# 0Setsuna0/SoftbodyUnity

Measured on AMD Instinct MI355X. Metric: particle-substeps/sec, higher is better.
Workload: dtype f32

## Files before the change

include/softbody_debug.h:

```cpp
#ifndef SOFTBODY_MI355X_DEBUG_H
#define SOFTBODY_MI355X_DEBUG_H

#include "softbody.h"

#ifdef __cplusplus
extern "C" {
#endif

#define SB_DEBUG_NO_COMM  1u
#define SB_DEBUG_LOOPBACK 2u

#define SB_TUNE_NO_MASS_PALETTE   (1u << 0)
#define SB_TUNE_NO_UNIFORM_MASS   (1u << 1)
#define SB_TUNE_NO_PALETTE        (1u << 2)
#define SB_TUNE_NO_WAVE_ITEMS     (1u << 3)
#define SB_TUNE_NO_LANE_PACK      (1u << 4)
#define SB_TUNE_NO_COST_ORDER     (1u << 5)
#define SB_TUNE_NO_FUSED_UNPACK   (1u << 6)
#define SB_TUNE_PEER_COARSE       (1u << 7)
#define SB_TUNE_NO_LAZY_TICK      (1u << 8)
#define SB_TUNE_NO_PACK           (1u << 9)
#define SB_TUNE_NO_PEEK           (1u << 10)
#define SB_TUNE_NO_KIN_FUSE       (1u << 11)
#define SB_TUNE_NO_WIDE_SLOTS     (1u << 12)
#define SB_TUNE_AUTO_PREFER_OVERLAP (1u << 13)
#define SB_TUNE_NO_AUTO_CALIBRATION (1u << 14)
typedef struct {
    uint32_t flags;
    int32_t tile_lanes;
    int32_t quad_lanes;
    int32_t narrow_min_tiles;
    int32_t store_through_max_tiles;
    int32_t store_through_large;
    int32_t peek_min_tiles;
    int32_t lds_pad_bytes;
    int32_t win_dwords;
    int32_t prev_offset_bytes;
    int32_t reserved[6];
} sb_tuning;
void sb_tuning_default(sb_tuning *t);
int sb_set_tuning(sb_solver *s, const sb_tuning *t);

int sb_profile_begin(sb_solver *s);
int sb_profile_end(sb_solver *s, float *elapsed_ms_out);
int sb_step_profiled(sb_solver *s, float dt, int32_t substeps, float *slot_ms_out, int32_t *slot_launches_out,
                     int32_t n_slots);
typedef struct {
    int64_t exchanges;
    double pack_ms, transport_ms, total_ms;
    double exposed_wait_ms;
} sb_exchange_timing;
int sb_debug_exchange_timing(sb_solver *s, int32_t enabled);
int sb_debug_exchange_timing_read(sb_solver *s, sb_exchange_timing *out);

int sb_debug_launch(sb_solver *s, float dt, int32_t substeps, int32_t it, int32_t gcolour);
int sb_debug_halo_pack(sb_solver *s, int32_t slot, float *host_out, int64_t capacity_floats, int64_t *count_floats_out);
int sb_debug_halo_unpack(sb_solver *s, int32_t slot, const float *host_in, int64_t count_floats);

typedef struct {
    int64_t tiles_checked, groups_checked, constraints_checked;
    int64_t errors[6];
    int32_t first_stage;
    int32_t first_tile, first_group, first_kind;
} sb_validate_report;
int sb_debug_validate(sb_solver *s, int32_t inject_fault, sb_validate_report *out);

int sb_debug_last_words(int32_t fd, const char *text, int64_t len, int32_t exit_code);

#ifdef __cplusplus
}
#endif
#endif
```

softbodyunity_amd/csrc/abi.hip:

```cpp
#include "solver_internal.hpp"

using namespace sbi;

extern "C" {

void sb_desc_default(sb_desc *d) {
    if (!d) return;
    std::memset(d, 0, sizeof(*d));
    d->world = 1;
    d->gravity[1] = -9.81f;
    d->tile_particles = 0;
    d->use_graph = 1;
}

int sb_create(const sb_desc *desc, sb_solver **out) {
    if (!desc || !out) return fail(SB_ERR_INVALID_ARG, "sb_create: null argument");
    *out = nullptr;
    return guarded([&]() -> int {
        sb_desc d = *desc;
        if (d.world <= 0) d.world = 1;
        if (d.rank < 0 || d.rank >= d.world) return fail(SB_ERR_INVALID_ARG, "sb_create: rank out of range");
        if (!(d.damping >= 0.0f)) return fail(SB_ERR_INVALID_ARG, "sb_create: damping must be >= 0");
        if (d.tile_particles > sbp::kMaxTileLocal) return fail(SB_ERR_INVALID_ARG, "sb_create: tile_particles too large");
        if (d.partition < SB_PARTITION_AUTO || d.partition > SB_PARTITION_RCB) return fail(SB_ERR_INVALID_ARG, "sb_create: partition must be SB_PARTITION_AUTO, _BLOCKS or _RCB");
        if (d.plan_flags & ~kPlanFlagsAll) return fail(SB_ERR_INVALID_ARG, "sb_create: unknown bit in plan_flags");
        if (d.halo_transport != SB_TRANSPORT_RCCL && d.halo_transport != SB_TRANSPORT_PEER) return fail(SB_ERR_INVALID_ARG, "sb_create: halo_transport must be SB_TRANSPORT_RCCL or _PEER");
        if (d.halo_schedule < SB_SCHEDULE_AUTO || d.halo_schedule > SB_SCHEDULE_OVERLAP_GRAPH) return fail(SB_ERR_INVALID_ARG, "sb_create: halo_schedule must be one of SB_SCHEDULE_*");
        if (d.debug_flags & ~(SB_DEBUG_NO_COMM | SB_DEBUG_LOOPBACK)) return fail(SB_ERR_INVALID_ARG, "sb_create: unknown bit in debug_flags");
        if (d.reserved[0] || d.reserved[1] || d.reserved[2]) return fail(SB_ERR_INVALID_ARG, "sb_create: reserved fields must be 0 (zero-initialise sb_desc or call sb_desc_default)");
        int ndev = 0;
        hipError_t e = hipGetDeviceCount(&ndev);
        if (e != hipSuccess || ndev <= 0)
            return fail(SB_ERR_NO_DEVICE, "sb_create: no HIP device (this plugin has no CPU path)");
        if (d.device < 0 || d.device >= ndev) return fail(SB_ERR_NO_DEVICE, "sb_create: device ordinal out of range");
        hipDeviceProp_t prop;
        HIP_CHECK(hipGetDeviceProperties(&prop, d.device));
        if (std::strncmp(prop.gcnArchName, "gfx950", 6) != 0)
            return fail(SB_ERR_NO_DEVICE, std::string("sb_create: device is ") + prop.gcnArchName + ", kernels are built for gfx950 only");
        HIP_CHECK(hipSetDevice(d.device));
        auto s = std::make_unique<sb_solver>();
        s->desc = d;
        s->peer.enabled = d.world > 1 && d.halo_transport == SB_TRANSPORT_PEER;
        s->loopback = d.world > 1 && (d.debug_flags & SB_DEBUG_LOOPBACK) != 0;
        HIP_CHECK(hipStreamCreateWithFlags(&s->stream, hipStreamNonBlocking));
        HIP_CHECK(hipEventCreate(&s->ev0));
        HIP_CHECK(hipEventCreate(&s->ev1));
        *out = s.release();
        return SB_OK;
    });
}

void sb_tuning_default(sb_tuning *t) {
    if (!t) return;
    std::memset(t, 0, sizeof(*t));
    t->store_through_max_tiles = -1;
    t->peek_min_tiles = -1;
}

int sb_set_tuning(sb_solver *s, const sb_tuning *t) {
    if (!s || !t) return fail(SB_ERR_INVALID_ARG, "sb_set_tuning: null argument");
    if (s->finalized) return fail(SB_ERR_STATE, "sb_set_tuning after sb_finalize");
    constexpr uint32_t kAll = (SB_TUNE_NO_AUTO_CALIBRATION << 1) - 1u;
    if (t->flags & ~kAll) return fail(SB_ERR_INVALID_ARG, "sb_set_tuning: unknown bit in flags");
    for (int32_t r : t->reserved) if (r) return fail(SB_ERR_INVALID_ARG, "sb_set_tuning: reserved fields must be 0 (sb_tuning_default)");
    if (t->tile_lanes != 0 && t->tile_lanes != 128 && t->tile_lanes != 256 && t->tile_lanes != 512) return fail(SB_ERR_INVALID_ARG, "sb_set_tuning: tile_lanes must be 0, 128, 256 or 512");
    if (t->quad_lanes != 0 && t->quad_lanes != 256 && t->quad_lanes != 512) return fail(SB_ERR_INVALID_ARG, "sb_set_tuning: quad_lanes must be 0, 256 or 512");
    if (t->prev_offset_bytes < 0 || (t->prev_offset_bytes & 15)) return fail(SB_ERR_INVALID_ARG, "sb_set_tuning: prev_offset_bytes must be a non-negative multiple of 16");
    if (t->narrow_min_tiles < 0 || t->store_through_max_tiles < -1 || t->peek_min_tiles < -1 || t->lds_pad_bytes < 0 || t->win_dwords < 0 || (t->store_through_large & ~3))
        return fail(SB_ERR_INVALID_ARG, "sb_set_tuning: value out of range");
    s->tune_flags = t->flags;
    s->lazy_tick = !(t->flags & SB_TUNE_NO_LAZY_TICK);
    s->pack_tiles = !(t->flags & SB_TUNE_NO_PACK);
    s->peek_enabled = !(t->flags & SB_TUNE_NO_PEEK);
    s->kin_fuse = !(t->flags & SB_TUNE_NO_KIN_FUSE);
    s->tile_lanes = t->tile_lanes;
    s->quad_lanes = t->quad_lanes ? t->quad_lanes : 512;
    if (t->narrow_min_tiles > 0) s->narrow_min_tiles = t->narrow_min_tiles;
    if (t->store_through_max_tiles >= 0) s->store_through_max_tiles = t->store_through_max_tiles;
    s->store_through_large = t->store_through_large;
    if (t->peek_min_tiles >= 0) s->peek_min_tiles = t->peek_min_tiles;
    s->lds_pad = (size_t)t->lds_pad_bytes;
    s->win_dwords_cap = t->win_dwords;
    s->prev_offset_bytes = t->prev_offset_bytes;
    return SB_OK;
}

int sb_destroy(sb_solver *s) {
    if (!s) return fail(SB_ERR_INVALID_ARG, "sb_destroy: null handle");
    (void)hipSetDevice(s->desc.device);
    delete s;
    return SB_OK;
}

int sb_set_particles(sb_solver *s, const float *pos, const float *vel, const float *inv_mass, int32_t n) {
    if (!s || !pos || !inv_mass || n <= 0) return fail(SB_ERR_INVALID_ARG, "sb_set_particles: bad argument");
    if (s->finalized) return fail(SB_ERR_STATE, "sb_set_particles after sb_finalize");
    return guarded([&]() -> int {
        for (int32_t p = 0; p < n; ++p) if (!(inv_mass[p] >= 0.0f)) return fail(SB_ERR_INVALID_ARG, "sb_set_particles: inverse mass must be >= 0");
        s->n = n;
        s->pos.assign(pos, pos + 3 * (size_t)n);
        if (vel) s->vel.assign(vel, vel + 3 * (size_t)n); else s->vel.assign(3 * (size_t)n, 0.0f);
        s->invm.assign(inv_mass, inv_mass + n);
        return SB_OK;
    });
}

int sb_set_rest_positions(sb_solver *s, const float *rest, int32_t n) {
    if (!s || !rest) return fail(SB_ERR_INVALID_ARG, "sb_set_rest_positions: bad argument");
    if (s->finalized) return fail(SB_ERR_STATE, "sb_set_rest_positions after sb_finalize");
    if (n != s->n) return fail(SB_ERR_INVALID_ARG, "sb_set_rest_positions: n differs from sb_set_particles");
    return guarded([&]() -> int { s->rest.assign(rest, rest + 3 * (size_t)n); return SB_OK; });
}

static int set_cons(sb_solver *s, const char *who, const int32_t *idx, const float *rest, int32_t m, float compliance,
                    int type, int nv, int nrest) {
// ... 274 lines not shown
    return SB_OK;
}

int finalize_agree(sb_solver *s, int local_rc) {
    const int W = s->desc.world;
    const size_t rec = (size_t)W + 2;
    const std::string my_error = local_rc ? std::string(last_error_text()) : std::string();
    std::vector<uint64_t> mine = agreement_record(s, local_rc != SB_OK);
    std::vector<uint64_t> all((size_t)W * rec);
    const int rc = guarded([&]() -> int {
        int r0 = set_device(s); if (r0) return r0;
        DevBuf<uint64_t> d_all; int64_t acct = 0;
        d_all.alloc((size_t)W * rec, acct);
        HIP_CHECK(hipMemcpy(d_all.p + (size_t)s->desc.rank * rec, mine.data(), rec * sizeof(uint64_t), hipMemcpyHostToDevice));
        NCCL_CHECK(rccl().AllGather(d_all.p + (size_t)s->desc.rank * rec, d_all.p, rec * sizeof(uint64_t), ncclUint8, s->comm, s->stream));
        HIP_CHECK(hipStreamSynchronize(s->stream));
        HIP_CHECK(hipMemcpy(all.data(), d_all.p, all.size() * sizeof(uint64_t), hipMemcpyDeviceToHost));
        return SB_OK;
    });
    if (local_rc) return fail(local_rc, my_error);
    if (rc) return rc;
    return check_agreement(all, W, s->desc.rank);
}

int finalize_link(sb_solver *s) {
    return guarded([&]() -> int {
        int rc = set_device(s); if (rc) return rc;
        if (s->peer.enabled && s->desc.world > 1) {
            if (s->loopback) {
                peer_link(s);
            } else if (s->comm) {
                const int W = s->desc.world;
                hipIpcMemHandle_t mine;
                HIP_CHECK(hipIpcGetMemHandle(&mine, s->peer.mailbox));
                DevBuf<uint8_t> d_all; int64_t acct = 0;
                d_all.alloc((size_t)W * sizeof(mine), acct);
                HIP_CHECK(hipMemcpy(d_all.p + (size_t)s->desc.rank * sizeof(mine), &mine, sizeof(mine), hipMemcpyHostToDevice));
                NCCL_CHECK(rccl().AllGather(d_all.p + (size_t)s->desc.rank * sizeof(mine), d_all.p, sizeof(mine), ncclUint8, s->comm, s->stream));
                HIP_CHECK(hipStreamSynchronize(s->stream));
                std::vector<hipIpcMemHandle_t> all((size_t)W);
                HIP_CHECK(hipMemcpy(all.data(), d_all.p, (size_t)W * sizeof(mine), hipMemcpyDeviceToHost));
                for (int r = 0; r < W; ++r) {
                    if (r == s->desc.rank) continue;
                    bool needed = false;
                    for (const auto &H : s->halos) for (int pr : H->peers) needed |= pr == r;
                    if (!needed) continue;
                    void *p = nullptr;
                    HIP_CHECK(hipIpcOpenMemHandle(&p, all[(size_t)r], hipIpcMemLazyEnablePeerAccess));
                    s->peer.remote[(size_t)r] = (uint32_t *)p; s->peer.opened[(size_t)r] = 1;
                }
                peer_link(s);
            }
        }
        if (std::getenv("SB_PRINT_ALLOC"))
            std::fprintf(stderr, "[alloc] pos3 %p prev %p vel %p wf %p w8 %p T0.stream %p T1.stream %p T0.tiles %p T1.tiles %p\n", (void *)s->d_pos3.p, (void *)s->d_prev.p,
                         (void *)s->d_vel.p, (void *)s->d_wf.p, (void *)s->d_w8.p, (void *)s->tiling[0].stream.p, (void *)s->tiling[1].stream.p,
                         (void *)s->tiling[0].tiles.p, (void *)s->tiling[1].tiles.p);
        HIP_CHECK(hipDeviceSynchronize());
        std::vector<float>().swap(s->pos); std::vector<float>().swap(s->vel); std::vector<float>().swap(s->rest);
        std::vector<int32_t>().swap(s->dist_ij); std::vector<int32_t>().swap(s->vol_ijkl); std::vector<int32_t>().swap(s->bend_ijkl);
        std::vector<float>().swap(s->dist_rest); std::vector<float>().swap(s->vol_rest); std::vector<float>().swap(s->bend_rest);
        s->finalized = true;
        return SB_OK;
    });
}

}

extern "C" {

int sb_finalize(sb_solver *s) {
    if (!s) return fail(SB_ERR_INVALID_ARG, "sb_finalize: null handle");
    if (s->finalized) return fail(SB_ERR_STATE, "sb_finalize called twice");
    if (s->n <= 0) return fail(SB_ERR_STATE, "sb_finalize before sb_set_particles");
    const bool no_comm = (s->desc.debug_flags & SB_DEBUG_NO_COMM) != 0;
    if (s->desc.world > 1 && !s->comm && !s->peer.enabled && !no_comm)
        return fail(SB_ERR_STATE, "sb_finalize: world > 1 needs sb_comm_init first (or halo_transport = SB_TRANSPORT_PEER with sb_peer_connect)");
    int rc = guarded([&]() -> int { return finalize_local(s); });
    if (s->desc.world > 1 && s->comm && !s->loopback) rc = finalize_agree(s, rc);
    if (rc) return rc;
    return finalize_link(s);
}

int sb_synchronize(sb_solver *s) {
    if (!s) return fail(SB_ERR_INVALID_ARG, "sb_synchronize: null handle");
    return guarded([&]() -> int {
        int rc = set_device(s); if (rc) return rc;
        flush_deferred(s);
        HIP_CHECK(hipStreamSynchronize(s->stream));
        check_peer_error(s);
        return SB_OK;
    });
}

int sb_get_owner(sb_solver *s, int32_t *owner, int32_t n) {
    if (!s || !owner) return fail(SB_ERR_INVALID_ARG, "sb_get_owner: null argument");
    if (!s->finalized) return fail(SB_ERR_STATE, "sb_get_owner before sb_finalize");
    if (n != s->n) return fail(SB_ERR_INVALID_ARG, "sb_get_owner: n mismatch");
    std::memcpy(owner, s->plan->plan.owner_of_old.data(), (size_t)n * sizeof(int32_t));
    return SB_OK;
}

int sb_profile_begin(sb_solver *s) {
    if (!s) return fail(SB_ERR_INVALID_ARG, "sb_profile_begin: null handle");
    return guarded([&]() -> int {
        int rc = set_device(s); if (rc) return rc;
        HIP_CHECK(hipEventRecord(s->ev0, s->stream));
        return SB_OK;
    });
}
// ... 78 lines not shown
```

softbodyunity_amd/csrc/solver_internal.hpp:

```cpp
#pragma once
#include <hip/hip_runtime.h>
#include <rccl/rccl.h>
#include <dlfcn.h>

#include <algorithm>
#include <array>
#include <atomic>
#include <chrono>
#include <climits>
#include <cmath>
#include <cstdio>
#include <cstdlib>
#include <cstring>
#include <limits>
#include <map>
#include <memory>
#include <mutex>
#include <type_traits>
#include <stdexcept>
#include <string>
#include <utility>
#include <vector>

#include "../../include/softbody.h"
// ... 32 lines not shown
    decltype(&ncclGroupEnd) GroupEnd = nullptr;
    decltype(&ncclSend) Send = nullptr;
    decltype(&ncclRecv) Recv = nullptr;
    decltype(&ncclAllGather) AllGather = nullptr;
    bool ok() const { return handle != nullptr; }
};
RcclApi &rccl(bool required = true);
#define NCCL_CHECK(expr)                                                                                  \
    do {                                                                                                  \
        ncclResult_t r_ = (expr);                                                                         \
        if (r_ != ncclSuccess)                                                                            \
            throw HipError(SB_ERR_RCCL, std::string(#expr) + ": " + rccl().GetErrorString(r_));          \
    } while (0)

int hip_runtime_version();
bool capture_overlap_ok();

template <class T>
struct DevBuf {
    T *p = nullptr;
    T *base = nullptr;
    size_t count = 0;
    DevBuf() = default;
    DevBuf(const DevBuf &) = delete;
    DevBuf &operator=(const DevBuf &) = delete;
    DevBuf(DevBuf &&o) noexcept : p(o.p), base(o.base), count(o.count) { o.p = o.base = nullptr; o.count = 0; }
    DevBuf &operator=(DevBuf &&o) noexcept { if (this != &o) { free(); p = o.p; base = o.base; count = o.count; o.p = o.base = nullptr; o.count = 0; } return *this; }
    void alloc(size_t n, int64_t &acct, size_t lead_elems = 0) {
        free();
        count = n;
        if (n) { HIP_CHECK(hipMalloc((void **)&base, (n + lead_elems) * sizeof(T))); p = base + lead_elems; acct += (int64_t)((n + lead_elems) * sizeof(T)); }
    }
    void upload(const std::vector<T> &h, int64_t &acct) {
        alloc(h.size(), acct);
        if (!h.empty()) HIP_CHECK(hipMemcpy(p, h.data(), h.size() * sizeof(T), hipMemcpyHostToDevice));
    }
    void free() { if (base) { (void)hipFree(base); } base = nullptr; p = nullptr; count = 0; }
    ~DevBuf() { free(); }
};

struct DevHalo {
    std::vector<int> peers;
    std::vector<int32_t> send_off, recv_off;
    DevBuf<int32_t> send_idx, recv_idx;
    bool active() const { return !peers.empty(); }
};

struct DevTiling {
    int32_t n_tiles = 0;
    size_t lds_bytes = 0;
    int64_t n_slots = 0;
    int64_t staged_particles = 0;
    int64_t stream_bytes = 0;
    int32_t max_local = 0, win_dwords = 4, pal_dwords = 0, rounds_dwords = 0;
    int32_t n_boundary = 0;
    bool has_quads = false;
    int32_t item_waves = 0;
    int32_t packed_lanes = 0;
    int64_t n_packed_tiles = 0;
    DevBuf<sbk::TileDesc> tiles;
    DevBuf<int2> runs_overflow;
    DevBuf<uint32_t> stream;
    DevBuf<int32_t> gather;
};

struct DevGColour {
    int type = 0;
    int32_t count = 0;
    DevBuf<int2> ij;
    DevBuf<int4> quad;
    DevBuf<float> rest;
    DevBuf<float2> rest2;
};

}

namespace sbi {

enum class StepKind : uint8_t { Tile, T2Layer, GColour, Exchange, ForkExchange, JoinExchange };
enum class TileRange : uint8_t { All, T0Boundary, T0Interior, T1Interior, T1Boundary };
struct TickStep {
    StepKind kind;
    TileRange range;
    bool kin;
    int it, substeps;
    int index;
};
struct TickShape { int substeps; bool fuse, defer_last, kin; };

struct ExchangeTimer {
    bool enabled = false;
    std::vector<hipEvent_t> pending, join_pending, free_list;
    void mark(hipStream_t st, bool join = false);
    ~ExchangeTimer();
};

}

using sbi::DevBuf; using sbi::DevGColour; using sbi::DevHalo; using sbi::DevTiling;

struct sb_plan {
    sbp::Plan plan;
    sbp::LocalPlan local;
    bool owns_local = true;
};

// ... 230 lines not shown
```

softbodyunity_amd/csrc/tables.hip:

```cpp
#include "solver_internal.hpp"

namespace sbi {

sbp::Input make_input(const float *rest, int32_t n, const int32_t *d, int64_t md, const int32_t *v, int64_t mv,
                      const int32_t *b, int64_t mb) {
    sbp::Input in;
    in.rest = rest; in.n = n; in.dist_ij = d; in.m_d = md; in.vol = v; in.m_v = mv; in.bend = b; in.m_b = mb;
    return in;
}

sbp::Domain to_domain(const sb_domain &d) {
    sbp::Domain D;
    D.set = true; D.n_global = d.n_global; D.ell = d.spacing; D.fill = d.fill > 0 && d.fill <= 1 ? d.fill : 1.0;
    for (int a = 0; a < 3; ++a) { D.lo[a] = d.lo[a]; D.hi[a] = d.hi[a]; }
    return D;
}
sbp::Opts plan_opts(int rank, int world, const int32_t dims[3], int32_t tile_particles, int32_t partition, uint32_t plan_flags,
                    int64_t m_v, int64_t m_b, const sb_domain *domain) {
    sbp::Opts o;
    if (domain) {
        o.domain = to_domain(*domain);
        if (domain->four_vertex_constraints) m_v += 1;
    }
    o.rank = rank; o.world = world <= 0 ? 1 : world;
// ... 410 lines not shown
                        } else {
                            stream.push_back(idx);
                            stream.push_back(rb);
                        }
                    }
                }
                while ((stream.size() - s0) & 3) stream.push_back(0);
                for (int t = 1; t < 3; ++t)
                    for (const Part &pt : R.parts) {
                        const uint32_t b = (uint32_t)base[pt.member], b2 = b | (b << 16);
                        const int64_t kb = pt.first_q + (t == 2 ? pt.cnt[1] : 0);
                        for (int64_t k = kb; k < kb + pt.cnt[t]; ++k) {
                            if (G.t_quad_type[k] != t) throw std::runtime_error("internal: group layout");
                            Q.has_quads = true;
                            stream.push_back(G.t_quad[2 * k] + b2); stream.push_back(G.t_quad[2 * k + 1] + b2);
                            const int32_t id = G.t_quad_id[k];
                            if (t == 1) { volatile float r6 = 6.0f * s->vol_rest[id]; stream.push_back(fbits(r6)); stream.push_back(0); }
                            else { stream.push_back(fbits(s->bend_rest[2 * (size_t)id])); stream.push_back(fbits(s->bend_rest[2 * (size_t)id + 1])); }
                        }
                    }
            }
            td.s_len = (uint32_t)(stream.size() - s0);
            if (!td.packed_lanes) max_data = std::max(max_data, td.s_len - td.s_hdr);
            tiles.push_back(td);
        }
        });
        std::vector<sbk::TileDesc> tiles;
        std::vector<int2> overflow;
        std::vector<uint32_t> stream;
        std::vector<int32_t> dev_gather;
        int32_t max_local = 0, max_pal = 0, max_rounds = 0;
        uint32_t max_data = 4;
        {
            size_t nt = 0, no = 0, ns = 0, ng = 0;
            for (const Piece &Q : pieces) { nt += Q.tiles.size(); no += Q.overflow.size(); ns += Q.stream.size(); ng += Q.dev_gather.size(); }
            if (ns > 0xfffffff0ull) throw std::runtime_error("tile constraint stream exceeds 2^32 dwords");
            tiles.reserve(nt); overflow.reserve(no); stream.reserve(ns); dev_gather.reserve(ng);
            for (Piece &Q : pieces) {
                for (sbk::TileDesc td : Q.tiles) {
                    td.s_begin += (uint32_t)stream.size();
                    td.run_overflow += (int32_t)overflow.size();
                    td.gather_begin += (int32_t)dev_gather.size();
                    tiles.push_back(td);
                }
                overflow.insert(overflow.end(), Q.overflow.begin(), Q.overflow.end());
                stream.insert(stream.end(), Q.stream.begin(), Q.stream.end());
                dev_gather.insert(dev_gather.end(), Q.dev_gather.begin(), Q.dev_gather.end());
                max_local = std::max(max_local, Q.max_local); max_pal = std::max(max_pal, Q.max_pal);
                max_rounds = std::max(max_rounds, Q.max_rounds); max_data = std::max(max_data, Q.max_data);
                D.has_quads |= Q.has_quads;
                Piece().tiles.swap(Q.tiles); std::vector<uint32_t>().swap(Q.stream);
            }
        }
        if (!(s->tune_flags & SB_TUNE_NO_COST_ORDER)) {
            constexpr int32_t kCostOrderMaxTiles = 2048;
            const int32_t n = (int32_t)tiles.size();
            std::vector<std::pair<int32_t, int32_t>> ranges;
            if (tl == 2) ranges = s->t2_layer_range;
            else if ((s->overlap_halo || s->calib.state == 1) && D.n_boundary > 0 && D.n_boundary < n) {
                const int32_t cut = tl == 0 ? D.n_boundary : n - D.n_boundary;
                ranges = {{0, cut}, {cut, n}};
            } else ranges = {{0, n}};
            for (const auto &rg : ranges) {
                const int32_t nr = rg.second - rg.first;
                if (nr < 2 || nr > kCostOrderMaxTiles) continue;
                std::vector<int32_t> cost((size_t)nr), idx((size_t)nr);
                for (int32_t k = 0; k < nr; ++k) {
                    const sbk::TileDesc &td = tiles[(size_t)(rg.first + k)];
                    int32_t c = 0;
                    for (int32_t r = 0; r < td.n_rounds; ++r) {
                        const uint32_t w = stream[(size_t)td.s_begin + (size_t)r];
                        const int32_t nd = (int32_t)(w & 1023u), nv = (int32_t)((w >> 10) & 1023u), nb = (int32_t)((w >> 20) & 1023u);
                        if (D.has_quads) {
                            const int nw = std::max(1, (int)D.item_waves ? (int)D.item_waves : 4);
                            c += std::max(1, (((nd + 63) >> 6) + ((nv + 15) >> 4) + ((nb + 3) >> 2) + nw - 1) / nw) + (nb > 0 ? 1 : 0);
                        }
                        else c += std::max(1, (nd + sbk::kRoundSlots - 1) / sbk::kRoundSlots);
                    }
                    cost[(size_t)k] = c; idx[(size_t)k] = k;
                }
                const auto mm = std::minmax_element(cost.begin(), cost.end());
                if ((int64_t)*mm.second * 4 <= (int64_t)*mm.first * 5) continue;
                std::stable_sort(idx.begin(), idx.end(), [&](int32_t a, int32_t b2) { return cost[(size_t)a] > cost[(size_t)b2]; });
                std::vector<sbk::TileDesc> placed((size_t)nr);
                const int32_t xq = nr >> 3, xr = nr & 7;
                for (int32_t w = 0; w < nr; ++w) {
                    const int32_t xcd = w & 7;
                    const int32_t pos = (xcd < xr ? xcd * (xq + 1) : xr * (xq + 1) + (xcd - xr) * xq) + (w >> 3);
                    placed[(size_t)pos] = tiles[(size_t)(rg.first + idx[(size_t)w])];
                }
                std::copy(placed.begin(), placed.end(), tiles.begin() + rg.first);
            }
        }
        D.n_tiles = (int32_t)tiles.size();
        D.n_packed_tiles = n_packed_tiles.load();
        D.max_local = std::max(max_local, 1);
        D.win_dwords = (int32_t)std::min<uint32_t>(max_data, 8192u);
        if (s->win_dwords_cap > 0) D.win_dwords = std::max(1024, std::min(D.win_dwords, s->win_dwords_cap) & ~3);
        D.pal_dwords = (max_pal + 3) & ~3;
        D.rounds_dwords = std::min(sbk::kMaxRoundsLds, (max_rounds + 3) & ~3);
        D.lds_bytes = (size_t)D.max_local * sizeof(float4) + (size_t)D.rounds_dwords * 4 + (size_t)D.pal_dwords * 4 + (size_t)D.win_dwords * 4 + 16;
        D.n_slots = 0;
        for (size_t ci = 0; ci < LT.tile_ids.size(); ++ci) {
            const sbp::Tile &T = G.tiles[LT.tile_ids[ci]];
            D.n_slots += (T.d_end - T.d_begin) + (T.q_end - T.q_begin);
        }
        D.staged_particles = 0;
        for (const sbk::TileDesc &td : tiles) D.staged_particles += td.n_local;
        D.stream_bytes = (int64_t)stream.size() * 4;
        D.tiles.upload(tiles, s->dev_bytes); D.runs_overflow.upload(overflow, s->dev_bytes);
        D.stream.upload(stream, s->dev_bytes);
        D.gather.upload(dev_gather, s->dev_bytes);
    }
    for (const sbp::LocalGColour &LG : L.gcolours) {
        auto D = std::make_unique<DevGColour>();
        D->type = LG.type; D->count = (int32_t)LG.id.size();
        if (LG.type == 0) {
            std::vector<int2> ij(LG.id.size()); std::vector<float> rest(LG.id.size());
            for (size_t k = 0; k < LG.id.size(); ++k) { ij[k] = make_int2(LG.idx[2 * k], LG.idx[2 * k + 1]); rest[k] = s->dist_rest[LG.id[k]]; }
            D->ij.upload(ij, s->dev_bytes); D->rest.upload(rest, s->dev_bytes);
        } else {
            std::vector<int4> q(LG.id.size()); std::vector<float2> rest(LG.id.size());
            for (size_t k = 0; k < LG.id.size(); ++k) {
                q[k] = make_int4(LG.idx[4 * k], LG.idx[4 * k + 1], LG.idx[4 * k + 2], LG.idx[4 * k + 3]);
                const int32_t id = LG.id[k];
                if (LG.type == 1) { volatile float r6 = 6.0f * s->vol_rest[id]; rest[k] = make_float2(r6, 0.0f); }
                else rest[k] = make_float2(s->bend_rest[2 * (size_t)id], s->bend_rest[2 * (size_t)id + 1]);
            }
            D->quad.upload(q, s->dev_bytes); D->rest2.upload(rest, s->dev_bytes);
        }
        s->gcolours.push_back(std::move(D));
    }
    size_t max_send = 0, max_recv = 0;
    for (size_t slot = 0; slot < L.halo.size(); ++slot) {
        const sbp::HaloSlot &H = L.halo[slot];
        auto D = std::make_unique<DevHalo>();
        std::vector<int32_t> sidx, ridx;
        D->send_off.push_back(0); D->recv_off.push_back(0);
        for (int peer = 0; peer < L.world; ++peer) {
            if (H.send_idx[peer].empty() && H.recv_idx[peer].empty()) continue;
            D->peers.push_back(peer);
            sidx.insert(sidx.end(), H.send_idx[peer].begin(), H.send_idx[peer].end());
            ridx.insert(ridx.end(), H.recv_idx[peer].begin(), H.recv_idx[peer].end());
            D->send_off.push_back((int32_t)sidx.size()); D->recv_off.push_back((int32_t)ridx.size());
        }
        D->send_idx.upload(sidx, s->dev_bytes); D->recv_idx.upload(ridx, s->dev_bytes);
        const size_t fl = slot == 1 ? 6 : 3;
        max_send = std::max(max_send, sidx.size() * fl); max_recv = std::max(max_recv, ridx.size() * fl);
        s->halos.push_back(std::move(D));
    }
    s->d_sendbuf.alloc(max_send, s->dev_bytes);
    s->d_recvbuf.alloc(max_recv, s->dev_bytes);
    if (max_recv) HIP_CHECK(hipMemset(s->d_recvbuf.p, 0, max_recv * sizeof(float)));
    s->fused_unpack = false;
    if (L.world > 1 && !s->peer.enabled && P.tiling && P.gcolours.empty() && P.t2_layers.empty() && !s->tiling[1].has_quads &&
        s->halos.size() > 1 && !(s->tune_flags & SB_TUNE_NO_FUSED_UNPACK)) {
        std::vector<int32_t> ridx;
        for (int peer = 0; peer < L.world; ++peer) ridx.insert(ridx.end(), L.halo[1].recv_idx[(size_t)peer].begin(), L.halo[1].recv_idx[(size_t)peer].end());
        bool identity = (int64_t)ridx.size() == s->n_local - s->n_owned && !ridx.empty();
        for (size_t k = 0; identity && k < ridx.size(); ++k) identity = ridx[k] == (int32_t)(s->n_owned + (int64_t)k);
        s->fused_unpack = identity;
    }
// ... 45 lines not shown
```

softbodyunity_amd/native.py:

```python
import ctypes as C
import os

import numpy as np

_HERE = os.path.dirname(os.path.abspath(__file__))
_VARIANT = os.environ.get("SB_LIB_VARIANT", "")
LIB_PATH = os.path.join(_HERE, f"libsoftbody_mi355x{'_' + _VARIANT if _VARIANT else ''}.so")

SB_UNIQUE_ID_BYTES = 128
SB_IPC_HANDLE_BYTES = 64
SB_OK = 0
SB_PARTITION_AUTO, SB_PARTITION_BLOCKS, SB_PARTITION_RCB = 0, 1, 2
SB_PLAN_NO_T2, SB_PLAN_NO_THIRD_LIST, SB_PLAN_NO_CLUSTER_LAYERS, SB_PLAN_NO_MIXED_GROUPS, SB_PLAN_NO_BANK_ORDER, SB_PLAN_NO_TILE_MERGE = 1, 2, 4, 8, 16, 32
SB_TRANSPORT_RCCL, SB_TRANSPORT_PEER = 0, 1
SB_SCHEDULE_AUTO, SB_SCHEDULE_SERIAL_EAGER, SB_SCHEDULE_SERIAL_GRAPH, SB_SCHEDULE_OVERLAP_EAGER, SB_SCHEDULE_OVERLAP_GRAPH = 0, 1, 2, 3, 4
SB_DEBUG_NO_COMM, SB_DEBUG_LOOPBACK = 1, 2
SB_GROUP_WALK = 1
SB_GROUP_WHOLE_MESH = 2
(SB_TUNE_NO_MASS_PALETTE, SB_TUNE_NO_UNIFORM_MASS, SB_TUNE_NO_PALETTE, SB_TUNE_NO_WAVE_ITEMS, SB_TUNE_NO_LANE_PACK, SB_TUNE_NO_COST_ORDER,
 SB_TUNE_NO_FUSED_UNPACK, SB_TUNE_PEER_COARSE, SB_TUNE_NO_LAZY_TICK, SB_TUNE_NO_PACK, SB_TUNE_NO_PEEK, SB_TUNE_NO_KIN_FUSE,
 SB_TUNE_NO_WIDE_SLOTS, SB_TUNE_AUTO_PREFER_OVERLAP, SB_TUNE_NO_AUTO_CALIBRATION) = (1 << k for k in range(15))
SB_ERR_INVALID_ARG, SB_ERR_STATE, SB_ERR_NO_DEVICE, SB_ERR_HIP, SB_ERR_RCCL, SB_ERR_NOMEM, SB_ERR_UNSUPPORTED = \
    -1, -2, -3, -4, -5, -6, -7


class SbDesc(C.Structure):
    _fields_ = [("device", C.c_int32), ("rank", C.c_int32), ("world", C.c_int32), ("part_dims", C.c_int32 * 3),
                ("gravity", C.c_float * 3), ("damping", C.c_float), ("tile_particles", C.c_int32),
                ("use_graph", C.c_int32), ("partition", C.c_int32), ("plan_flags", C.c_uint32),
                ("halo_transport", C.c_int32), ("halo_schedule", C.c_int32), ("debug_flags", C.c_uint32),
                ("reserved", C.c_int32 * 3)]


class SbTuning(C.Structure):
    _fields_ = [("flags", C.c_uint32), ("tile_lanes", C.c_int32), ("quad_lanes", C.c_int32), ("narrow_min_tiles", C.c_int32),
                ("store_through_max_tiles", C.c_int32), ("store_through_large", C.c_int32), ("peek_min_tiles", C.c_int32),
                ("lds_pad_bytes", C.c_int32), ("win_dwords", C.c_int32), ("prev_offset_bytes", C.c_int32), ("reserved", C.c_int32 * 6)]


class SbExchangeTiming(C.Structure):
    _fields_ = [("exchanges", C.c_int64), ("pack_ms", C.c_double), ("transport_ms", C.c_double), ("total_ms", C.c_double), ("exposed_wait_ms", C.c_double)]


class SbStats(C.Structure):
    _fields_ = [("n_particles_owned", C.c_int64), ("n_particles_local", C.c_int64),
                ("n_constraints_local", C.c_int64 * 3), ("n_tilings", C.c_int32), ("n_global_colours", C.c_int32),
                ("n_tiles", C.c_int64 * 2), ("tile_constraints", C.c_int64 * 2), ("constraints_in_tiles", C.c_int64),
                ("constraints_in_global", C.c_int64), ("halo_particles_t1", C.c_int64),
                ("halo_particles_global", C.c_int64), ("device_bytes", C.c_int64),
                ("n_t2_layers", C.c_int64), ("n_t2_tiles", C.c_int64), ("t2_constraints", C.c_int64),
                ("launch_bytes", C.c_int64 * 5), ("partition", C.c_int32), ("halo_peers", C.c_int32),
                ("partition_cost", C.c_int64), ("partition_cost_max", C.c_int64), ("partition_cost_total", C.c_int64),
                ("halo_particles_recv", C.c_int64), ("plan_hash", C.c_uint64), ("halo_schedule", C.c_int32),
                ("halo_unpack_fused", C.c_int32), ("readback_peeks", C.c_int64), ("readback_peek_tiles", C.c_int64), ("ticks_fused", C.c_int64), ("ticks_fused_kinematic", C.c_int64), ("lane_packed_tiles", C.c_int64 * 2),
                ("halo_auto_state", C.c_int32), ("halo_auto_ticks", C.c_int32), ("halo_auto_ms", C.c_double * 2)]

    def as_dict(self):
        out = {}
        for name, _ in self._fields_:
            v = getattr(self, name)
            out[name] = list(v) if hasattr(v, "__len__") else v
        return out


class SbValidateReport(C.Structure):
    _fields_ = [("tiles_checked", C.c_int64), ("groups_checked", C.c_int64), ("constraints_checked", C.c_int64), ("errors", C.c_int64 * 6),
                ("first_stage", C.c_int32), ("first_tile", C.c_int32), ("first_group", C.c_int32), ("first_kind", C.c_int32)]


class SbDomain(C.Structure):
    _fields_ = [("n_global", C.c_int64), ("lo", C.c_double * 3), ("hi", C.c_double * 3), ("spacing", C.c_double), ("fill", C.c_double),
                ("four_vertex_constraints", C.c_int32), ("reserved", C.c_int32)]


# ... 131 lines not shown
        _lib = L
    return _lib


def check(rc):
    if rc != SB_OK:
        raise SoftbodyError(rc, lib().sb_last_error().decode("utf-8", "replace"))


def ptr(a):
    return None if a is None else a.ctypes.data_as(C.c_void_p)


def f32(a, shape=None):
    a = np.ascontiguousarray(a, dtype=np.float32)
    return a if shape is None else a.reshape(shape)


def i32(a, shape=None):
    a = np.ascontiguousarray(a, dtype=np.int32)
    return a if shape is None else a.reshape(shape)


_PLAN_FLAG_ENV = (("SB_NO_T2", SB_PLAN_NO_T2), ("SB_NO_THIRD_LIST", SB_PLAN_NO_THIRD_LIST),
                  ("SB_NO_CLUSTER_LAYERS", SB_PLAN_NO_CLUSTER_LAYERS), ("SB_NO_MIXED_GROUPS", SB_PLAN_NO_MIXED_GROUPS),
                  ("SB_NO_BANK_ORDER", SB_PLAN_NO_BANK_ORDER), ("SB_NO_TILE_MERGE", SB_PLAN_NO_TILE_MERGE))


def plan_flags_from_env():
    lists = int(os.environ.get("SB_BALANCED_LISTS", "0") or 0) & 3
    return sum(bit for name, bit in _PLAN_FLAG_ENV if os.environ.get(name)) | (lists << 8)


def halo_transport_from_env():
    return SB_TRANSPORT_PEER if os.environ.get("SB_HALO_TRANSPORT") == "peer" else SB_TRANSPORT_RCCL


def halo_schedule_from_env():
    overlap, graph = bool(os.environ.get("SB_HALO_OVERLAP")), bool(os.environ.get("SB_GRAPH_RCCL"))
    if not overlap and not graph:
        return SB_SCHEDULE_AUTO
    return (SB_SCHEDULE_OVERLAP_GRAPH if graph else SB_SCHEDULE_OVERLAP_EAGER) if overlap else SB_SCHEDULE_SERIAL_GRAPH


def debug_flags_from_env():
    return (SB_DEBUG_NO_COMM if os.environ.get("SB_TEST_NO_COMM") else 0) | (SB_DEBUG_LOOPBACK if os.environ.get("SB_TEST_LOOPBACK") else 0)


_TUNE_FLAG_ENV = (("SB_NO_MASS_PALETTE", SB_TUNE_NO_MASS_PALETTE), ("SB_NO_UNIFORM_MASS", SB_TUNE_NO_UNIFORM_MASS), ("SB_NO_PALETTE", SB_TUNE_NO_PALETTE),
                  ("SB_NO_WAVE_ITEMS", SB_TUNE_NO_WAVE_ITEMS), ("SB_NO_LANE_PACK", SB_TUNE_NO_LANE_PACK), ("SB_NO_COST_ORDER", SB_TUNE_NO_COST_ORDER),
                  ("SB_NO_FUSED_UNPACK", SB_TUNE_NO_FUSED_UNPACK), ("SB_PEER_COARSE", SB_TUNE_PEER_COARSE), ("SB_NO_LAZY_TICK", SB_TUNE_NO_LAZY_TICK),
                  ("SB_NO_PACK", SB_TUNE_NO_PACK), ("SB_NO_PEEK", SB_TUNE_NO_PEEK), ("SB_NO_KIN_FUSE", SB_TUNE_NO_KIN_FUSE),
                  ("SB_NO_WIDE_SLOTS", SB_TUNE_NO_WIDE_SLOTS), ("SB_AUTO_PREFER_OVERLAP", SB_TUNE_AUTO_PREFER_OVERLAP),
                  ("SB_NO_AUTO_CALIBRATION", SB_TUNE_NO_AUTO_CALIBRATION))
_TUNE_INT_ENV = (("SB_TILE_LANES", "tile_lanes"), ("SB_QUAD_LANES", "quad_lanes"), ("SB_NARROW_MIN_TILES", "narrow_min_tiles"),
                 ("SB_STORE_THROUGH_MAX_TILES", "store_through_max_tiles"), ("SB_STORE_THROUGH_LARGE", "store_through_large"),
                 ("SB_PEEK_MIN_TILES", "peek_min_tiles"), ("SB_LDS_PAD", "lds_pad_bytes"), ("SB_WIN_DWORDS", "win_dwords"),
                 ("SB_PREV_OFFSET", "prev_offset_bytes"))


def tuning_from_env():
    t = SbTuning()
    lib().sb_tuning_default(C.byref(t))
    any_set = False
    for name, bit in _TUNE_FLAG_ENV:
        if os.environ.get(name):
            t.flags |= bit; any_set = True
    for name, field in _TUNE_INT_ENV:
        v = os.environ.get(name)
        if v not in (None, ""):
            setattr(t, field, int(v)); any_set = True
    return t if any_set else None


def runtime_info():
    ri = SbRuntimeInfo()
    check(lib().sb_runtime_info(C.byref(ri)))
    return {"hip_runtime_version": ri.hip_runtime_version, "hip_driver_version": ri.hip_driver_version,
            "rccl_version": ri.rccl_version, "rccl_header_version": ri.rccl_header_version,
            "rccl_was_resident": bool(ri.rccl_was_resident), "capture_serial_ok": bool(ri.capture_serial_ok),
            "capture_overlap_ok": bool(ri.capture_overlap_ok), "hip_library": ri.hip_library.decode(),
            "rccl_library": ri.rccl_library.decode()}


def domain_from_mesh(rest_pos, dist_ij=None, vol_ijkl=None, bend_ijkl=None):
    rest = f32(rest_pos, (-1, 3))
    d = i32(dist_ij if dist_ij is not None else np.zeros((0, 2)), (-1, 2))
    v = i32(vol_ijkl if vol_ijkl is not None else np.zeros((0, 4)), (-1, 4))
    b = i32(bend_ijkl if bend_ijkl is not None else np.zeros((0, 4)), (-1, 4))
    out = SbDomain()
    check(lib().sb_domain_from_mesh(ptr(rest), rest.shape[0], ptr(d), d.shape[0], ptr(v), v.shape[0], ptr(b), b.shape[0], C.byref(out)))
    return out


def make_domain(n_global, lo, hi, spacing, four_vertex_constraints=False):
    d = SbDomain()
    d.n_global = int(n_global); d.lo[:] = [float(c) for c in lo]; d.hi[:] = [float(c) for c in hi]
    d.spacing = float(spacing); d.fill = 1.0; d.four_vertex_constraints = 1 if four_vertex_constraints else 0
    return d


def domain_window(domain, rank, world, part_dims=(0, 0, 0), tile_particles=0):
    o = SbPlanOpts(rank, world, (C.c_int32 * 3)(*part_dims), tile_particles, SB_PARTITION_BLOCKS, 0, None, None)
    lo = (C.c_double * 3)(); hi = (C.c_double * 3)()
    check(lib().sb_domain_window(C.byref(domain), C.byref(o), lo, hi))
    return np.array(lo[:]), np.array(hi[:])

# ... 114 lines not shown
```

Measured before the change: 107.3 billion.

## Deduplicate identical tile constraint programs into a shared stream

At setup, each tile's instruction stream is hashed and compared, and tiles with byte-identical programs (same header, length and words) are pointed at a single shared copy. Shared programs are placed first in the new stream. The aim is a smaller stream footprint, so tiles reading the same program hit in cache instead of fetching distinct copies from memory. The cost is extra host-side hashing and sorting at finalize. A flag is added to disable it, along with diagnostic output.

After: 113.7 billion (median of 6 runs). +5.9%, better.

```diff
diff --git a/include/softbody_debug.h b/include/softbody_debug.h
--- a/include/softbody_debug.h
+++ b/include/softbody_debug.h
@@ -25,6 +25,7 @@
 #define SB_TUNE_NO_WIDE_SLOTS     (1u << 12)
 #define SB_TUNE_AUTO_PREFER_OVERLAP (1u << 13)
 #define SB_TUNE_NO_AUTO_CALIBRATION (1u << 14)
+#define SB_TUNE_NO_SHARED_PROGRAMS (1u << 15)
 typedef struct {
     uint32_t flags;
     int32_t tile_lanes;
diff --git a/softbodyunity_amd/csrc/abi.hip b/softbodyunity_amd/csrc/abi.hip
--- a/softbodyunity_amd/csrc/abi.hip
+++ b/softbodyunity_amd/csrc/abi.hip
@@ -60,7 +60,7 @@
 int sb_set_tuning(sb_solver *s, const sb_tuning *t) {
     if (!s || !t) return fail(SB_ERR_INVALID_ARG, "sb_set_tuning: null argument");
     if (s->finalized) return fail(SB_ERR_STATE, "sb_set_tuning after sb_finalize");
-    constexpr uint32_t kAll = (SB_TUNE_NO_AUTO_CALIBRATION << 1) - 1u;
+    constexpr uint32_t kAll = (SB_TUNE_NO_SHARED_PROGRAMS << 1) - 1u;
     if (t->flags & ~kAll) return fail(SB_ERR_INVALID_ARG, "sb_set_tuning: unknown bit in flags");
     for (int32_t r : t->reserved) if (r) return fail(SB_ERR_INVALID_ARG, "sb_set_tuning: reserved fields must be 0 (sb_tuning_default)");
     if (t->tile_lanes != 0 && t->tile_lanes != 128 && t->tile_lanes != 256 && t->tile_lanes != 512) return fail(SB_ERR_INVALID_ARG, "sb_set_tuning: tile_lanes must be 0, 128, 256 or 512");
@@ -441,10 +441,17 @@
                 peer_link(s);
             }
         }
-        if (std::getenv("SB_PRINT_ALLOC"))
+        if (std::getenv("SB_PRINT_ALLOC")) {
             std::fprintf(stderr, "[alloc] pos3 %p prev %p vel %p wf %p w8 %p T0.stream %p T1.stream %p T0.tiles %p T1.tiles %p\n", (void *)s->d_pos3.p, (void *)s->d_prev.p,
                          (void *)s->d_vel.p, (void *)s->d_wf.p, (void *)s->d_w8.p, (void *)s->tiling[0].stream.p, (void *)s->tiling[1].stream.p,
                          (void *)s->tiling[0].tiles.p, (void *)s->tiling[1].tiles.p);
+            for (int tl = 0; tl < 3; ++tl) {
+                const DevTiling &D = s->tiling[tl];
+                if (D.n_tiles)
+                    std::fprintf(stderr, "[alloc] T%d: %d tiles, %lld distinct programs, stream %lld B read by the tiles, %lld B uploaded\n", tl, D.n_tiles,
+                                 (long long)D.n_programs, (long long)D.stream_bytes, (long long)(D.stream.count * sizeof(uint32_t)));
+            }
+        }
         HIP_CHECK(hipDeviceSynchronize());
         std::vector<float>().swap(s->pos); std::vector<float>().swap(s->vel); std::vector<float>().swap(s->rest);
         std::vector<int32_t>().swap(s->dist_ij); std::vector<int32_t>().swap(s->vol_ijkl); std::vector<int32_t>().swap(s->bend_ijkl);
diff --git a/softbodyunity_amd/csrc/solver_internal.hpp b/softbodyunity_amd/csrc/solver_internal.hpp
--- a/softbodyunity_amd/csrc/solver_internal.hpp
+++ b/softbodyunity_amd/csrc/solver_internal.hpp
@@ -108,6 +108,7 @@
     int64_t n_slots = 0;
     int64_t staged_particles = 0;
     int64_t stream_bytes = 0;
+    int64_t n_programs = 0;
     int32_t max_local = 0, win_dwords = 4, pal_dwords = 0, rounds_dwords = 0;
     int32_t n_boundary = 0;
     bool has_quads = false;
diff --git a/softbodyunity_amd/csrc/tables.hip b/softbodyunity_amd/csrc/tables.hip
--- a/softbodyunity_amd/csrc/tables.hip
+++ b/softbodyunity_amd/csrc/tables.hip
@@ -486,6 +486,59 @@
                 Piece().tiles.swap(Q.tiles); std::vector<uint32_t>().swap(Q.stream);
             }
         }
+        D.stream_bytes = (int64_t)stream.size() * 4;
+        D.n_programs = (int64_t)tiles.size();
+        if (!(s->tune_flags & SB_TUNE_NO_SHARED_PROGRAMS) && tiles.size() > 1) {
+            const size_t nt = tiles.size();
+            std::vector<uint64_t> key(nt);
+            sbp::parallel_for_chunks((int64_t)nt, 1024, [&](int64_t, int64_t tb, int64_t te) {
+                for (int64_t t = tb; t < te; ++t) {
+                    const sbk::TileDesc &td = tiles[(size_t)t];
+                    if (td.s_len & 3u) throw std::runtime_error("internal: tile stream not 16-byte aligned");
+                    uint64_t h = 1469598103934665603ull;
+                    h = (h ^ td.s_hdr) * 1099511628211ull;
+                    h = (h ^ td.s_len) * 1099511628211ull;
+                    const uint32_t *w = stream.data() + td.s_begin;
+                    for (uint32_t k = 0; k < td.s_len; ++k) h = (h ^ w[k]) * 1099511628211ull;
+                    key[(size_t)t] = h;
+                }
+            });
+            std::vector<int32_t> by_key(nt);
+            for (size_t t = 0; t < nt; ++t) by_key[t] = (int32_t)t;
+            std::sort(by_key.begin(), by_key.end(), [&](int32_t a, int32_t b) { return key[(size_t)a] != key[(size_t)b] ? key[(size_t)a] < key[(size_t)b] : a < b; });
+            auto same = [&](int32_t a, int32_t b) {
+                const sbk::TileDesc &x = tiles[(size_t)a], &y = tiles[(size_t)b];
+                return x.s_hdr == y.s_hdr && x.s_len == y.s_len &&
+                       std::memcmp(stream.data() + x.s_begin, stream.data() + y.s_begin, (size_t)x.s_len * 4) == 0;
+            };
+            std::vector<int32_t> rep(nt), uses(nt, 0);
+            std::vector<int32_t> reps;
+            for (size_t g0 = 0, g1; g0 < nt; g0 = g1) {
+                for (g1 = g0 + 1; g1 < nt && key[(size_t)by_key[g1]] == key[(size_t)by_key[g0]]; ++g1) {}
+                reps.clear();
+                for (size_t q = g0; q < g1; ++q) {
+                    const int32_t t = by_key[q];
+                    int32_t r = t;
+                    for (int32_t c : reps) if (same(c, t)) { r = c; break; }
+                    if (r == t) reps.push_back(t);
+                    rep[(size_t)t] = r; ++uses[(size_t)r];
+                }
+            }
+            std::vector<uint32_t> shared;
+            std::vector<uint32_t> at(nt, 0u);
+            int64_t n_programs = 0;
+            for (int pass = 0; pass < 2; ++pass)
+                for (size_t t = 0; t < nt; ++t)
+                    if (rep[t] == (int32_t)t && (uses[t] > 1) == (pass == 0)) {
+                        at[t] = (uint32_t)shared.size();
+                        const uint32_t *w = stream.data() + tiles[t].s_begin;
+                        shared.insert(shared.end(), w, w + tiles[t].s_len);
+                        ++n_programs;
+                    }
+            for (size_t t = 0; t < nt; ++t) tiles[t].s_begin = at[(size_t)rep[t]];
+            stream.swap(shared);
+            D.n_programs = n_programs;
+        }
         if (!(s->tune_flags & SB_TUNE_NO_COST_ORDER)) {
             constexpr int32_t kCostOrderMaxTiles = 2048;
             const int32_t n = (int32_t)tiles.size();
@@ -541,7 +594,6 @@
         }
         D.staged_particles = 0;
         for (const sbk::TileDesc &td : tiles) D.staged_particles += td.n_local;
-        D.stream_bytes = (int64_t)stream.size() * 4;
         D.tiles.upload(tiles, s->dev_bytes); D.runs_overflow.upload(overflow, s->dev_bytes);
         D.stream.upload(stream, s->dev_bytes);
         D.gather.upload(dev_gather, s->dev_bytes);
diff --git a/softbodyunity_amd/native.py b/softbodyunity_amd/native.py
--- a/softbodyunity_amd/native.py
+++ b/softbodyunity_amd/native.py
@@ -19,7 +19,7 @@
 SB_GROUP_WHOLE_MESH = 2
 (SB_TUNE_NO_MASS_PALETTE, SB_TUNE_NO_UNIFORM_MASS, SB_TUNE_NO_PALETTE, SB_TUNE_NO_WAVE_ITEMS, SB_TUNE_NO_LANE_PACK, SB_TUNE_NO_COST_ORDER,
  SB_TUNE_NO_FUSED_UNPACK, SB_TUNE_PEER_COARSE, SB_TUNE_NO_LAZY_TICK, SB_TUNE_NO_PACK, SB_TUNE_NO_PEEK, SB_TUNE_NO_KIN_FUSE,
- SB_TUNE_NO_WIDE_SLOTS, SB_TUNE_AUTO_PREFER_OVERLAP, SB_TUNE_NO_AUTO_CALIBRATION) = (1 << k for k in range(15))
+ SB_TUNE_NO_WIDE_SLOTS, SB_TUNE_AUTO_PREFER_OVERLAP, SB_TUNE_NO_AUTO_CALIBRATION, SB_TUNE_NO_SHARED_PROGRAMS) = (1 << k for k in range(16))
 SB_ERR_INVALID_ARG, SB_ERR_STATE, SB_ERR_NO_DEVICE, SB_ERR_HIP, SB_ERR_RCCL, SB_ERR_NOMEM, SB_ERR_UNSUPPORTED = \
     -1, -2, -3, -4, -5, -6, -7
 
@@ -257,7 +257,7 @@
                   ("SB_NO_FUSED_UNPACK", SB_TUNE_NO_FUSED_UNPACK), ("SB_PEER_COARSE", SB_TUNE_PEER_COARSE), ("SB_NO_LAZY_TICK", SB_TUNE_NO_LAZY_TICK),
                   ("SB_NO_PACK", SB_TUNE_NO_PACK), ("SB_NO_PEEK", SB_TUNE_NO_PEEK), ("SB_NO_KIN_FUSE", SB_TUNE_NO_KIN_FUSE),
                   ("SB_NO_WIDE_SLOTS", SB_TUNE_NO_WIDE_SLOTS), ("SB_AUTO_PREFER_OVERLAP", SB_TUNE_AUTO_PREFER_OVERLAP),
-                  ("SB_NO_AUTO_CALIBRATION", SB_TUNE_NO_AUTO_CALIBRATION))
+                  ("SB_NO_AUTO_CALIBRATION", SB_TUNE_NO_AUTO_CALIBRATION), ("SB_NO_SHARED_PROGRAMS", SB_TUNE_NO_SHARED_PROGRAMS))
 _TUNE_INT_ENV = (("SB_TILE_LANES", "tile_lanes"), ("SB_QUAD_LANES", "quad_lanes"), ("SB_NARROW_MIN_TILES", "narrow_min_tiles"),
                  ("SB_STORE_THROUGH_MAX_TILES", "store_through_max_tiles"), ("SB_STORE_THROUGH_LARGE", "store_through_large"),
                  ("SB_PEEK_MIN_TILES", "peek_min_tiles"), ("SB_LDS_PAD", "lds_pad_bytes"), ("SB_WIN_DWORDS", "win_dwords"),
```
